# daeheepark/TrajSDE

Measured on AMD Instinct MI355X. Metric: scenes/sec (K=6, 20 SDE steps, ~256 agents) at 1/2/4/8 MI355X; minADE match, higher is better.
Workload: dtype f32 (fp16x3 split: 22-bit operands on v_mfma_f32_16x16x32_f16, f32 accumulate)

## Files before the change

### trajsde_amd/csrc/prep.hip

```cpp

#include <algorithm>
#include <cmath>
#include <limits>
#include <atomic>
#include <cstdlib>
#include <cstring>

#include "common.hpp"
#include "philox.hpp"
#include "tile.hpp"

namespace tsde {

__global__ void k_rotate(const float* __restrict__ ang, int N, const float* __restrict__ y, int F,
                         float* __restrict__ rot, float* __restrict__ y_rot) {
  const int per = F > 0 && y != nullptr ? F : 1;
  const int64_t idx = int64_t(blockIdx.x) * blockDim.x + threadIdx.x;
  if (idx >= int64_t(N) * per) return;
  const int i = int(idx / per), t = int(idx - int64_t(i) * per);
  const float s = sinf(ang[i]), c = cosf(ang[i]);
  if (t == 0) {
    f4 r = {c, -s, s, c};
    *reinterpret_cast<f4*>(rot + 4 * i) = r;
  }
  if (y != nullptr && F > 0) {
    const float a = y[(int64_t(i) * F + t) * 2], b = y[(int64_t(i) * F + t) * 2 + 1];
    y_rot[(int64_t(i) * F + t) * 2] = a * c + b * s;
    y_rot[(int64_t(i) * F + t) * 2 + 1] = b * c - a * s;
  }
}


constexpr int DONE_WAYS = 16;
__device__ __forceinline__ bool last_block_done(unsigned int* counters , unsigned int total) {
  __shared__ int s_last;
  asm volatile("s_waitcnt vmcnt(0)" ::: "memory");
  __syncthreads();
  if (threadIdx.x == 0) {
    const unsigned way = blockIdx.x % DONE_WAYS;
    const unsigned quota = total / DONE_WAYS + (way < total % DONE_WAYS ? 1u : 0u);
    int last = 0;
    if (__hip_atomic_fetch_add(&counters[way], 1u, __ATOMIC_RELAXED, __HIP_MEMORY_SCOPE_AGENT) + 1u == quota) {
      unsigned ways_used = total < unsigned(DONE_WAYS) ? total : unsigned(DONE_WAYS);
      last = __hip_atomic_fetch_add(&counters[DONE_WAYS], 1u, __ATOMIC_RELAXED, __HIP_MEMORY_SCOPE_AGENT) + 1u == ways_used;
    }
    s_last = last;
  }
  __syncthreads();
  return s_last != 0;
}
struct CoherentI32 {
  __amdgpu_buffer_rsrc_t rs;
  __device__ __forceinline__ explicit CoherentI32(const int32_t* base)
      : rs(__builtin_amdgcn_make_buffer_rsrc(const_cast<int32_t*>(base), 0, 0xFFFFFFFF, 0x00020000)) {}
  __device__ __forceinline__ int32_t operator[](int i) const { return __builtin_amdgcn_raw_buffer_load_b32(rs, i * 4, 0, 16 ); }
};
__device__ __forceinline__ void store_through(int32_t* p, int32_t v) { __hip_atomic_store(p, v, __ATOMIC_RELAXED, __HIP_MEMORY_SCOPE_AGENT); }

constexpr int EPT = 16;
__device__ __forceinline__ void degree_body(int blk, const int64_t* __restrict__ ei, int E, int32_t* __restrict__ deg) {
  int d[EPT];
#pragma unroll
  for (int u = 0; u < EPT; ++u) {
    const int e = (blk * EPT + u) * 256 + int(threadIdx.x);
    d[u] = e < E ? int(ei[int64_t(E) + e]) : -1;
  }
#pragma unroll
  for (int u = 0; u < EPT; ++u)
    if (d[u] >= 0) atomicAdd(&deg[d[u]], 1);
}
__device__ __forceinline__ void scatter_body(int blk, const int64_t* __restrict__ ei, int E, const int32_t* __restrict__ rowptr,
                                             int32_t* __restrict__ deg, int32_t* __restrict__ out) {
  int d[EPT], p[EPT], src[EPT];
#pragma unroll
  for (int u = 0; u < EPT; ++u) {
    const int e = (blk * EPT + u) * 256 + int(threadIdx.x);
    d[u] = e < E ? int(ei[int64_t(E) + e]) : -1;
    src[u] = e < E ? int32_t(ei[e]) : 0;
  }
#pragma unroll
  for (int u = 0; u < EPT; ++u) p[u] = d[u] >= 0 ? rowptr[d[u]] + atomicSub(&deg[d[u]], 1) - 1 : -1;
#pragma unroll
  for (int u = 0; u < EPT; ++u)
    if (p[u] >= 0) out[p[u]] = src[u];
}
__device__ __forceinline__ void scatter_lane_body(int blk, const int64_t* __restrict__ lai, int E, const int32_t* __restrict__ rowptr,
                                                  int32_t* __restrict__ deg, int64_t* __restrict__ out) {
  int d[EPT], p[EPT];
  int64_t key[EPT];
#pragma unroll
  for (int u = 0; u < EPT; ++u) {
    const int e = (blk * EPT + u) * 256 + int(threadIdx.x);
    d[u] = e < E ? int(lai[int64_t(E) + e]) : -1;
    key[u] = e < E ? ((lai[e] << 32) | int64_t(e)) : 0;
  }
#pragma unroll
  for (int u = 0; u < EPT; ++u) p[u] = d[u] >= 0 ? rowptr[d[u]] + atomicSub(&deg[d[u]], 1) - 1 : -1;
#pragma unroll
  for (int u = 0; u < EPT; ++u)
    if (p[u] >= 0) out[p[u]] = key[u];
}
__global__ __launch_bounds__(256) void k_scatter2(const int64_t* __restrict__ ei, int E, const int32_t* __restrict__ rowptr, int32_t* __restrict__ deg,
                                                  int32_t* __restrict__ csr_src, int nb_a, const int64_t* __restrict__ lai, int Ea,
                                                  const int32_t* __restrict__ la_rowptr, int32_t* __restrict__ la_deg, int64_t* __restrict__ la_pack) {
  const int blk = blockIdx.x;
  if (blk < nb_a) scatter_body(blk, ei, E, rowptr, deg, csr_src);
  else scatter_lane_body(blk - nb_a, lai, Ea, la_rowptr, la_deg, la_pack);
}
template <typename T, typename EMIT>
__device__ __forceinline__ void sort_long_rows(int vblk, int vgrid, const int32_t* __restrict__ rowptr, int n_rows, T* __restrict__ vals,
                                               T* buf , int32_t* __restrict__ low_out, int32_t* __restrict__ row_out,
                                               const EMIT& emit) {
  const T INF = sizeof(T) == 8 ? T(INT64_MAX) : T(INT32_MAX);
  for (int row = vblk; row < n_rows; row += vgrid) {
    const int beg = rowptr[row], n = rowptr[row + 1] - beg;
    if (n <= 256) continue;
    if (row_out != nullptr)
      for (int i = threadIdx.x; i < n; i += blockDim.x) row_out[beg + i] = row;
    int P = 2;
    while (P < n) P <<= 1;
    if (P <= 4096) {
      for (int i = threadIdx.x; i < P; i += blockDim.x) buf[i] = i < n ? vals[beg + i] : INF;
      __syncthreads();
      for (int k = 2; k <= P; k <<= 1)
        for (int j = k >> 1; j > 0; j >>= 1) {
          for (int i = threadIdx.x; i < P; i += blockDim.x) {
            const int l = i ^ j;
            if (l > i) {
              const T vi = buf[i], vl = buf[l];
              const bool up = (i & k) == 0;
              if ((vi > vl) == up) {
                buf[i] = vl;
                buf[l] = vi;
              }
            }
          }
          __syncthreads();
        }
      for (int i = threadIdx.x; i < n; i += blockDim.x) {
        vals[beg + i] = buf[i];
        if (low_out != nullptr) low_out[beg + i] = int32_t(int64_t(buf[i]) & 0xFFFFFFFFll);
        emit(beg + i, buf[i], row);
      }
      __syncthreads();
    } else {
      T* a = vals + beg;
      for (int k = 2; k <= P; k <<= 1)
        for (int j = k >> 1; j > 0; j >>= 1) {
          const int mask = (j == (k >> 1)) ? k - 1 : j;
          for (int i = threadIdx.x; i < n; i += blockDim.x) {
            const int l = i ^ mask;
            if (l > i && l < n) {
              const T vi = a[i], vl = a[l];
              if (vi > vl) {
                a[i] = vl;
                a[l] = vi;
              }
            }
          }
          __threadfence_block();
          __syncthreads();
        }
      for (int i = threadIdx.x; i < n; i += blockDim.x) {
        if (low_out != nullptr) low_out[beg + i] = int32_t(int64_t(a[i]) & 0xFFFFFFFFll);
        emit(beg + i, a[i], row);
      }
    }
  }
}

template <typename T>
__device__ __forceinline__ T lane_xor(T v, int mask) {
  if constexpr (sizeof(T) == 8) {
    const unsigned lo = unsigned(__shfl_xor(int(unsigned(v & 0xFFFFFFFFll)), mask)), hi = unsigned(__shfl_xor(int(unsigned((v >> 32) & 0xFFFFFFFFll)), mask));
    return T((int64_t(hi) << 32) | int64_t(lo));
  } else {
    return T(__shfl_xor(int(v), mask));
  }
}
template <typename T, typename EMIT>
__device__ __forceinline__ void row_sort_part(int vblk, int vgrid, const int32_t* __restrict__ rowptr, int n_rows, T* __restrict__ vals,
                                              int32_t* __restrict__ low_out ,
                                              int32_t* __restrict__ row_out ,
                                              T* buf , const EMIT& emit) {
  constexpr int EPL = 4, PMAX = 64 * EPL;
  const T INF = sizeof(T) == 8 ? T(INT64_MAX) : T(INT32_MAX);
  const int lane = threadIdx.x & 63, waves = blockDim.x >> 6;
  for (int row = vblk * waves + (threadIdx.x >> 6); row < n_rows; row += vgrid * waves) {
    const int beg = rowptr[row], n = rowptr[row + 1] - beg;
    if (n > PMAX) continue;
    if (row_out != nullptr) {
#pragma unroll
      for (int r = 0; r < EPL; ++r)
        if (64 * r + lane < n) row_out[beg + 64 * r + lane] = row;
    }
    if (n <= 1) {
      if (n == 1 && lane == 0) {
        const T v0 = vals[beg];
        if (low_out != nullptr) low_out[beg] = int32_t(int64_t(v0) & 0xFFFFFFFFll);
        emit(beg, v0, row);
      }
      continue;
    }
    T v[EPL];
#pragma unroll
    for (int r = 0; r < EPL; ++r) v[r] = EPL * lane + r < n ? vals[beg + EPL * lane + r] : INF;
#pragma unroll
    for (int k = 2; k <= PMAX; k <<= 1) {
      if ((k >> 1) >= n) break;
#pragma unroll
      for (int j = k >> 1; j > 0; j >>= 1) {
        if (j < EPL) {
#pragma unroll
          for (int r = 0; r < EPL; ++r) {
            const int l = r ^ j;
            if (l > r) {
              const bool up = ((EPL * lane + r) & k) == 0;
              const T a = v[r], b = v[l];
              const bool sw = (a > b) == up;
              v[r] = sw ? b : a;
              v[l] = sw ? a : b;
            }
          }
        } else {
          const int lj = j / EPL;
          const bool lower = (lane & lj) == 0;
#pragma unroll
          for (int r = 0; r < EPL; ++r) {
            const T o = lane_xor<T>(v[r], lj);
            const bool up = ((EPL * lane + r) & k) == 0;
            const bool keep_min = lower == up;
            v[r] = keep_min ? (o < v[r] ? o : v[r]) : (o > v[r] ? o : v[r]);
          }
        }
      }
    }
#pragma unroll
    for (int r = 0; r < EPL; ++r)
      if (EPL * lane + r < n) {
        vals[beg + EPL * lane + r] = v[r];
        if (low_out != nullptr) low_out[beg + EPL * lane + r] = int32_t(int64_t(v[r]) & 0xFFFFFFFFll);
        emit(beg + EPL * lane + r, v[r], row);
      }
  }
  sort_long_rows<T>(vblk, vgrid, rowptr, n_rows, vals, buf, low_out, row_out, emit);
}

__device__ __forceinline__ void ext_nodes_body(int i, int N, int A, int H, const int64_t* __restrict__ agent_index,
                                               const int64_t* __restrict__ batch, const int64_t* __restrict__ source,
                                               const uint8_t* __restrict__ bos, int32_t* __restrict__ orig, uint8_t* __restrict__ nus,
                                               int32_t* __restrict__ eos, int32_t* __restrict__ pick_slot) {
  __shared__ int32_t s_agents[256];
  int slot = -1;
  for (int k0 = 0; k0 < A; k0 += 256) {
    __syncthreads();
    s_agents[threadIdx.x] = k0 + int(threadIdx.x) < A ? int32_t(agent_index[k0 + threadIdx.x]) : -1;
    __syncthreads();
    const int m = A - k0 < 256 ? A - k0 : 256;
    if (i < N)
      for (int k = 0; k < m; ++k)
        if (s_agents[k] == i) slot = k0 + k;
  }
  if (i >= N + A) return;
  const int o = i < N ? i : int(agent_index[i - N]);
  orig[i] = o;
  nus[i] = (i < N ? source[batch[i]] : source[i - N]) == 0;
  int first = 0;
  {
    uint8_t bv[32];
#pragma unroll
    for (int t = 0; t < 32; ++t) bv[t] = bos[int64_t(o) * H + (t < H ? t : H - 1)];
#pragma unroll
    for (int t = 31; t >= 0; --t)
      if (t < H && bv[t]) first = t;
  }
  eos[i] = (H - 1) - first;
  pick_slot[i] = i < N ? slot : A + (i - N);
}

__device__ __forceinline__ void fake_x_body(int idx , int A, int H, const float* __restrict__ x,
                                            const int64_t* __restrict__ agent_index, const NoiseArg& na, float* __restrict__ x_fake) {
  const int quads = (2 * H + 3) / 4;
  if (idx >= A * quads) return;
  const int k = idx / quads, q = idx % quads;
  f4 z;
  if (na.z != nullptr) {
    for (int c = 0; c < 4; ++c) z[c] = (4 * q + c < 2 * H) ? na.z[int64_t(k) * 2 * H + 4 * q + c] : 0.f;
  } else {
    z = philox_normal4(noise_key(na), STREAM_FAKE_AGENT, 0u, na.row_ids ? uint32_t(na.row_ids[k]) : uint32_t(k), uint32_t(q));
  }
  const int64_t a = agent_index[k];
  for (int c = 0; c < 4; ++c) {
    const int col = 4 * q + c;
    if (col < 2 * H) x_fake[int64_t(k) * 2 * H + col] = x[a * 2 * H + col] + 2.0f * z[c];
  }
}

__device__ __forceinline__ float norm2_sq(float dx, float dy) { return fmaf(dy, dy, __fmul_rn(dx, dx)); }
__device__ __forceinline__ bool within_radius2(float dx, float dy, float thr2) { return norm2_sq(dx, dy) < thr2; }
static float radius2_threshold(float radius) {
  if (!(radius > 0.f)) return 0.f;
  if (std::isinf(radius)) return radius;
  float t = radius * radius;
  if (std::isinf(t)) t = std::numeric_limits<float>::max();
  while (t > 0.f && std::sqrt(t) >= radius) t = std::nextafter(t, 0.f);
  while (std::sqrt(t) < radius) t = std::nextafter(t, std::numeric_limits<float>::infinity());
  return t;
}

__device__ __forceinline__ void valid_mask_body(int i, int N, int H, int TT, const uint8_t* __restrict__ pad, uint32_t* __restrict__ vmask) {
  if (i >= N) return;
  uint32_t m = 0;
  uint8_t v[32];
#pragma unroll
  for (int t = 0; t < 32; ++t) v[t] = pad[int64_t(i) * TT + (t < H ? t : H - 1)];
#pragma unroll
  for (int t = 0; t < 32; ++t) m |= uint32_t(t < H && !v[t]) << t;
  vmask[i] = m;
}
__device__ __forceinline__ void time_major_body(int blk, int N, int H, int TT, const float* __restrict__ pos,
                                                const float* __restrict__ x, float2* __restrict__ pos_t, float2* __restrict__ x_t) {
  float2 pv[4], xv[4];
  int ii[4], tt[4];
#pragma unroll
  for (int u = 0; u < 4; ++u) {
    const int idx = (blk * 4 + u) * 256 + int(threadIdx.x);
    const bool live = idx < N * H;
    ii[u] = live ? idx / H : -1;
    tt[u] = live ? idx - ii[u] * H : 0;
    pv[u] = live ? reinterpret_cast<const float2*>(pos)[int64_t(ii[u]) * TT + tt[u]] : float2{0.f, 0.f};
    xv[u] = live ? reinterpret_cast<const float2*>(x)[int64_t(ii[u]) * H + tt[u]] : float2{0.f, 0.f};
  }
#pragma unroll
  for (int u = 0; u < 4; ++u)
    if (ii[u] >= 0) {
      pos_t[int64_t(tt[u]) * N + ii[u]] = pv[u];
      x_t[int64_t(tt[u]) * N + ii[u]] = xv[u];
    }
}

__device__ __forceinline__ void lane_feat_body(int l, int L, int P, const float* __restrict__ lp, const float* __restrict__ pad,
                                               float* __restrict__ feat) {
  if (l >= L) return;
  float len = 0.f;
  for (int j0 = 0; j0 < P; j0 += 8) {
    float pv[8];
#pragma unroll
    for (int u = 0; u < 8; ++u) pv[u] = pad[int64_t(l) * P + (j0 + u < P ? j0 + u : P - 1)];
#pragma unroll
    for (int u = 0; u < 8; ++u)
      if (j0 + u < P) len += 1.0f - pv[u];
  }
  int last = int(len - 1.0f);
  if (last < 0) last += P;
  feat[2 * l] = lp[(int64_t(l) * P + last) * 2] - lp[int64_t(l) * P * 2];
  feat[2 * l + 1] = lp[(int64_t(l) * P + last) * 2 + 1] - lp[int64_t(l) * P * 2 + 1];
}

__device__ __forceinline__ void block_scan_two(const int32_t* __restrict__ in0, int32_t* __restrict__ out0, const int32_t* __restrict__ in1,
                                               int32_t* __restrict__ out1, int n) {
  __shared__ int32_t s_w[2][4];
  __shared__ int32_t s_carry[2];
  constexpr int PT = 32;
  const int t = threadIdx.x, lane = t & 63, wv = t >> 6;
  if (t < 2) s_carry[t] = 0;
  __syncthreads();
  const CoherentI32 c0(in0), c1(in1);
  for (int base = 0; base < n; base += 256 * PT) {
    int32_t v[2][PT], sum[2] = {0, 0};
#pragma unroll
    for (int c = 0; c < PT; ++c) {
      const int i = base + PT * t + c;
      v[0][c] = i < n ? c0[i] : 0;
      v[1][c] = i < n ? c1[i] : 0;
    }
#pragma unroll
    for (int c = 0; c < PT; ++c) {
      sum[0] += v[0][c];
      sum[1] += v[1][c];
    }
    int32_t inc[2] = {sum[0], sum[1]};
#pragma unroll
    for (int d = 1; d < 64; d <<= 1) {
      const int32_t o0 = __shfl_up(inc[0], d), o1 = __shfl_up(inc[1], d);
      if (lane >= d) { inc[0] += o0; inc[1] += o1; }
    }
    if (lane == 63) { s_w[0][wv] = inc[0]; s_w[1][wv] = inc[1]; }
    __syncthreads();
#pragma unroll
    for (int a = 0; a < 2; ++a) {
      int32_t run = s_carry[a] + inc[a] - sum[a];
      for (int w = 0; w < wv; ++w) run += s_w[a][w];
      int32_t* out = a ? out1 : out0;
#pragma unroll
      for (int c = 0; c < PT; ++c) {
        const int i = base + PT * t + c;
        if (i < n) out[i] = run;
        run += v[a][c];
      }
    }
    __syncthreads();
    if (t < 2) s_carry[t] += s_w[t][0] + s_w[t][1] + s_w[t][2] + s_w[t][3];
    __syncthreads();
  }
}

struct FirstPassArgs {
  int N, A, H, TT, L, P, E, Ea, b0, b1, b2, b3, b4, b5, blocks;
  const int64_t *edge_index, *lane_actor_index, *agent_index, *batch, *source;
  const uint8_t *bos, *pad;
  const float *x, *pos, *lane_pos, *lane_pad;
  int32_t *deg, *la_deg, *rowptr, *la_rowptr, *orig, *eos, *pick_slot;
  uint8_t* nus;
  float *x_fake, *lane_feat;
  float2 *pos_t, *x_t;
  uint32_t* vmask;
  unsigned int* done;
  NoiseArg na;
};
__global__ __launch_bounds__(256) void k_prep_first(const FirstPassArgs a) {
  const int blk = blockIdx.x, i = threadIdx.x;
  if (blk < a.b0) degree_body(blk, a.edge_index, a.E, a.deg);
  else if (blk < a.b1) degree_body(blk - a.b0, a.lane_actor_index, a.Ea, a.la_deg);
  else if (blk < a.b2) ext_nodes_body((blk - a.b1) * 256 + i, a.N, a.A, a.H, a.agent_index, a.batch, a.source, a.bos, a.orig, a.nus, a.eos, a.pick_slot);
  else if (blk < a.b3) fake_x_body((blk - a.b2) * 256 + i, a.A, a.H, a.x, a.agent_index, a.na, a.x_fake);
  else if (blk < a.b4) valid_mask_body((blk - a.b3) * 256 + i, a.N, a.H, a.TT, a.pad, a.vmask);
  else if (blk < a.b5) time_major_body(blk - a.b4, a.N, a.H, a.TT, a.pos, a.x, a.pos_t, a.x_t);
  else lane_feat_body((blk - a.b5) * 256 + i, a.L, a.P, a.lane_pos, a.lane_pad, a.lane_feat);
  if (!last_block_done(a.done, unsigned(a.blocks))) return;
  block_scan_two(a.deg, a.rowptr, a.la_deg, a.la_rowptr, a.N + 1);
}

__global__ __launch_bounds__(256) void k_row_sort2(int N, int nb_a, int nb_l, const int32_t* __restrict__ rowptr, int32_t* __restrict__ csr_src,
                                                   int32_t* __restrict__ csr_dst, const uint32_t* __restrict__ vmask, int tref, int E,
                                                   uint8_t* __restrict__ flags_g, const int32_t* __restrict__ la_rowptr,
                                                   int64_t* __restrict__ la_pack, int32_t* __restrict__ la_eid, int32_t* __restrict__ la_actor,
                                                   const float* __restrict__ vec, float radius, int Ea, uint8_t* __restrict__ flags_la) {
  __shared__ int64_t buf[4096];
  const int blk = blockIdx.x;
  if (blk == 0 && threadIdx.x == 0) {
    flags_g[E] = 0;
    flags_la[Ea] = 0;
  }
  if (blk < nb_a) {
    if (E <= 0) return;
    auto emit = [&](int p, int32_t sender, int row) { flags_g[p] = uint8_t((vmask[sender] >> tref) & (vmask[row] >> tref) & 1u); };
    row_sort_part<int32_t>(blk, nb_a, rowptr, N, csr_src, nullptr, csr_dst, reinterpret_cast<int32_t*>(buf), emit);
  } else {
    if (Ea <= 0) return;
    auto emit = [&](int p, int64_t packed, int row) {
      (void)row;
      const int64_t e = packed & 0xFFFFFFFFll;
      flags_la[p] = uint8_t(sqrtf(norm2_sq(vec[2 * e], vec[2 * e + 1])) < radius);
    };
    row_sort_part<int64_t>(blk - nb_a, nb_l, la_rowptr, N, la_pack, la_eid, la_actor, buf, emit);
  }
}

constexpr int SCAN_MAX_BLOCKS = 512;
constexpr int SCAN_WORDS = SCAN_MAX_BLOCKS + 1;
constexpr int SCAN_INSTANCES = 3;
__device__ __forceinline__ int32_t lookback_prefix(unsigned long long* __restrict__ words, int b, int32_t total, int lane) {
  if (lane == 0)
    __hip_atomic_store(&words[b], ((b == 0 ? 2ull : 1ull) << 32) | (unsigned long long)(unsigned)total, __ATOMIC_RELAXED, __HIP_MEMORY_SCOPE_AGENT);
  int32_t prefix = 0;
  if (b > 0) {
    int j = b - 1;
    for (long spins = 0;; ++spins) {
      if (spins > (1L << 28)) __builtin_trap();
      const int k = j - lane;
      const unsigned long long w = k >= 0 ? __hip_atomic_load(&words[k], __ATOMIC_RELAXED, __HIP_MEMORY_SCOPE_AGENT) : (2ull << 32);
      const unsigned flag = unsigned(w >> 32);
      const unsigned long long done = __ballot(flag == 2u), none = __ballot(flag == 0u);
      const int upto = done ? __builtin_ctzll(done) : 63;
      const unsigned long long need = upto == 63 ? ~0ull : ((1ull << (upto + 1)) - 1);
      if (none & need) continue;
      int32_t part = lane <= upto ? int32_t(unsigned(w)) : 0;
#pragma unroll
      for (int d = 1; d < 64; d <<= 1) part += __shfl_xor(part, d);
      prefix += part;
      if (done) break;
      j -= 64;
    }
    if (lane == 0)
      __hip_atomic_store(&words[b], (2ull << 32) | (unsigned long long)(unsigned)(prefix + total), __ATOMIC_RELAXED, __HIP_MEMORY_SCOPE_AGENT);
  }
  return prefix;
}
struct ScanJob {
  const void* in;
  int32_t* out;
  int n, u8, blocks;
  unsigned long long* st;
};
struct ScanMultiArgs {
  ScanJob j[3];
  int njobs, blocks;
};
template <int PER>
__global__ __launch_bounds__(1024) void k_scan_multi(const ScanMultiArgs a) {
  __shared__ int32_t wsum[16];
  __shared__ int s_bid;
  __shared__ int32_t s_prefix;
  const int t = threadIdx.x, lane = t & 63, wv = t >> 6;
  int blk = blockIdx.x, q = 0;
  while (q + 1 < a.njobs && blk >= a.j[q].blocks) { blk -= a.j[q].blocks; ++q; }
  const ScanJob& job = a.j[q];
  const int n = job.n;
  if (t == 0) s_bid = int(__hip_atomic_fetch_add(&job.st[0], 1ull, __ATOMIC_RELAXED, __HIP_MEMORY_SCOPE_AGENT));
  __syncthreads();
  const int b = s_bid;
  const int64_t first = (int64_t(b) * 1024 + t) * PER;
  int32_t v[PER];
  int32_t s = 0;
#pragma unroll
  for (int i = 0; i < PER; ++i) {
    v[i] = first + i < n ? (job.u8 ? int32_t(static_cast<const uint8_t*>(job.in)[first + i]) : static_cast<const int32_t*>(job.in)[first + i]) : 0;
    s += v[i];
  }
  int32_t inc = s;
#pragma unroll
  for (int d = 1; d < 64; d <<= 1) {
    const int32_t o = __shfl_up(inc, d);
    if (lane >= d) inc += o;
  }
  if (lane == 63) wsum[wv] = inc;
  __syncthreads();
  int32_t wbase = 0;
  for (int w = 0; w < wv; ++w) wbase += wsum[w];
  if (wv == 0) {
    int32_t total = lane < 16 ? wsum[lane] : 0;
#pragma unroll
    for (int d = 1; d < 16; d <<= 1) total += __shfl_xor(total, d);
    total = __shfl(total, 0);
    const int32_t prefix = lookback_prefix(job.st + 1, b, total, lane);
    if (lane == 0) s_prefix = prefix;
  }
  __syncthreads();
  int32_t run = s_prefix + wbase + inc - s;
#pragma unroll
  for (int i = 0; i < PER; ++i) {
    if (first + i < n) job.out[first + i] = run;
    run += v[i];
  }
}
struct CollectArgs {
  int64_t n_aa;
  int E, Ea, N;
  const int32_t *aa_segptr, *cpos_g, *cpos_la, *rowptr, *la_rowptr;
  int32_t *g_segptr, *la_segptr, *counts;
  float radius, thr2;
  int radius_dev;
};
__device__ __forceinline__ void collect_body(int i, const CollectArgs& a) {
  if (i <= a.N) {
    a.g_segptr[i] = a.cpos_g[a.rowptr[i]];
    a.la_segptr[i] = a.cpos_la[a.la_rowptr[i]];
  }
  if (i == 0) {
    a.counts[0] = 0;
    a.counts[1] = a.aa_segptr[a.n_aa];
    a.counts[2] = a.cpos_g[a.E];
    a.counts[3] = a.cpos_la[a.Ea];
    if (!a.radius_dev) reinterpret_cast<float*>(a.counts)[4] = a.radius;
  }
}
__global__ void k_collect_counts(const CollectArgs a) { collect_body(blockIdx.x * blockDim.x + threadIdx.x, a); }

struct AaArgs {
  int N, Nt, H;
  float radius, thr2;
  int thr2_dev;
  const int32_t *rowptr, *csr_src, *orig;
  const uint32_t* vmask;
  const float2 *pos_t, *x_t;
  const float* rot;
  int32_t* segptr;
  int32_t* counts;
  unsigned long long* bal;
  int32_t *aa_dst, *aa_src;
  float* geom;
};
__device__ __forceinline__ int64_t bal_base(int row_start, int o) { return int64_t(row_start >> 6) + o; }
__device__ __forceinline__ int nth_set_bit(unsigned long long w, int r) {
  int posn = 0;
#pragma unroll
  for (int width = 32; width >= 1; width >>= 1) {
    const int c = __popcll((w >> posn) & ((1ull << width) - 1ull));
    if (r >= c) { r -= c; posn += width; }
  }
  return posn;
}
constexpr int AA_CG = 4, AA_SG = 7;
__global__ __launch_bounds__(256) void k_aa_count(const AaArgs a) {
  const int lane = threadIdx.x & 63;
  const int N = a.N, Nt = a.Nt, H = a.H;
  const int wid = __builtin_amdgcn_readfirstlane(int(xcd_block() * 4 + (threadIdx.x >> 6)));
  const int groups = (H + AA_SG - 1) / AA_SG, node = wid / groups, t0 = (wid - node * groups) * AA_SG;
  if (wid == 0 && lane == 0) {
    a.segptr[int64_t(H) * Nt] = 0;
    reinterpret_cast<float*>(a.counts)[4] = a.radius;
    reinterpret_cast<float*>(a.counts)[5] = a.thr2;
  }
  if (node >= Nt) return;
  const int o = node < N ? node : __builtin_amdgcn_readfirstlane(a.orig[node]);
  const int beg = __builtin_amdgcn_readfirstlane(a.rowptr[o]), end = __builtin_amdgcn_readfirstlane(a.rowptr[o + 1]);
  const uint32_t vo = __builtin_amdgcn_readfirstlane(a.vmask[o]);
  const int chunks = (end - beg + 63) >> 6;
  const int64_t bbase = bal_base(beg, o);
  const float thr2 = a.thr2;
  int mycnt = 0;
  for (int c0 = 0; c0 < chunks; c0 += AA_CG) {
    int s[AA_CG];
    uint32_t m[AA_CG];
#pragma unroll
    for (int u = 0; u < AA_CG; ++u) {
      const int p = beg + 64 * (c0 + u) + lane;
      s[u] = p < end ? a.csr_src[p] : -1;
    }
#pragma unroll
    for (int u = 0; u < AA_CG; ++u) {
      m[u] = s[u] >= 0 ? (a.vmask[s[u]] & vo) : 0u;
      s[u] = s[u] >= 0 ? s[u] : 0;
    }
    unsigned long long mine[AA_CG];
#pragma unroll
    for (int u = 0; u < AA_CG; ++u) mine[u] = 0ull;
    {
      float2 ps[AA_CG][AA_SG], pd[AA_SG];
#pragma unroll
      for (int q = 0; q < AA_SG; ++q) {
        const int t = t0 + q < H ? t0 + q : H - 1;
        pd[q] = a.pos_t[int64_t(t) * N + o];
#pragma unroll
        for (int u = 0; u < AA_CG; ++u) ps[u][q] = a.pos_t[int64_t(t) * N + s[u]];
      }
#pragma unroll
      for (int q = 0; q < AA_SG; ++q) {
        const int t = t0 + q;
        if (t >= H) break;
#pragma unroll
        for (int u = 0; u < AA_CG; ++u) {
          const bool ok = ((m[u] >> t) & 1u) && within_radius2(ps[u][q].x - pd[q].x, ps[u][q].y - pd[q].y, thr2);
          const unsigned long long B = __ballot(ok);
          mine[u] = lane == t ? B : mine[u];
        }
      }
    }
#pragma unroll
    for (int u = 0; u < AA_CG; ++u)
      if (c0 + u < chunks && lane >= t0 && lane < t0 + AA_SG && lane < H) {
        if (node < N) a.bal[(bbase + c0 + u) * H + lane] = mine[u];
        mycnt += __popcll(mine[u]);
      }
  }
  if (lane >= t0 && lane < t0 + AA_SG && lane < H) a.segptr[int64_t(lane) * Nt + node] = mycnt;
}
__device__ __forceinline__ void aa_fill_node(const AaArgs& a, int node, int part, int parts, int lane) {
  const int N = a.N, Nt = a.Nt, H = a.H;
  const int o = node < N ? node : __builtin_amdgcn_readfirstlane(a.orig[node]);
  const int beg = __builtin_amdgcn_readfirstlane(a.rowptr[o]), end = __builtin_amdgcn_readfirstlane(a.rowptr[o + 1]);
  if (end <= beg) return;
  const int chunks = (end - beg + 63) >> 6;
  const unsigned long long* __restrict__ words = a.bal + bal_base(beg, o) * H;
  int base_l = 0, n_l = 0;
  float2 pd_l = {0.f, 0.f};
  if (lane < H) {
    base_l = a.segptr[int64_t(lane) * Nt + node];
    n_l = a.segptr[int64_t(lane) * Nt + node + 1] - base_l;
    pd_l = a.pos_t[int64_t(lane) * N + o];
  }
  const int nw = chunks * H;
  const bool in_regs = nw <= 128;
  unsigned long long w0 = 0ull, w1 = 0ull;
  if (in_regs) {
    if (lane < nw) w0 = words[lane];
    if (64 + lane < nw) w1 = words[64 + lane];
  }
  const f4 R = *reinterpret_cast<const f4*>(a.rot + 4 * o);
  auto word = [&](int c, int t) -> unsigned long long {
    if (in_regs) {
      const int i = c * H + t;
      const unsigned long long src = i < 64 ? w0 : w1;
      const unsigned lo_ = __builtin_amdgcn_readlane(unsigned(src), i & 63), hi_ = __builtin_amdgcn_readlane(unsigned(src >> 32), i & 63);
      return (static_cast<unsigned long long>(hi_) << 32) | lo_;
    }
    return words[int64_t(c) * H + t];
  };
  for (int t = part; t < H; t += parts) {
    const int n = __builtin_amdgcn_readlane(n_l, t);
    if (n == 0) continue;
    const int64_t base = __builtin_amdgcn_readlane(base_l, t);
    const float pdx = __builtin_bit_cast(float, __builtin_amdgcn_readlane(__builtin_bit_cast(int, pd_l.x), t));
    const float pdy = __builtin_bit_cast(float, __builtin_amdgcn_readlane(__builtin_bit_cast(int, pd_l.y), t));
    const float2* __restrict__ pos_t = a.pos_t + int64_t(t) * N;
    const float2* __restrict__ x_t = a.x_t + int64_t(t) * N;
    const int seg = t * Nt + node;
    for (int r0 = 0; r0 < n; r0 += 64) {
      const int r = r0 + lane;
      unsigned long long selw = 0ull;
      int selc = 0, rr = 0, cum = 0;
      for (int c = 0; c < chunks; ++c) {
        const unsigned long long w = word(c, t);
        const int cc = __popcll(w);
        if (r >= cum && r < cum + cc) { selw = w; selc = c; rr = r - cum; }
        cum += cc;
        if (cum >= r0 + 64) break;
      }
      if (r < n) {
        const int sdr = a.csr_src[beg + 64 * selc + nth_set_bit(selw, rr)];
        const float2 ps = pos_t[sdr], xs = x_t[sdr];
        const float dx = ps.x - pdx, dy = ps.y - pdy;
        const float x0 = xs.x, x1 = xs.y;
        const f4 g = {x0 * R[0] + x1 * R[2], x0 * R[1] + x1 * R[3], dx * R[0] + dy * R[2], dx * R[1] + dy * R[3]};
        const int64_t k = base + r;
        *reinterpret_cast<f4*>(a.geom + 4 * k) = g;
        a.aa_dst[k] = seg;
        if (a.aa_src != nullptr) a.aa_src[k] = sdr;
      }
    }
  }
}

__device__ __forceinline__ void g_compact_body(int p, int E, int TT, int tref, const int32_t* __restrict__ csr_src, const int32_t* __restrict__ csr_dst,
                                               const float* __restrict__ pos, const float* __restrict__ rot, const float* __restrict__ ang,
                                               const uint8_t* __restrict__ flags, const int32_t* __restrict__ cpos, int32_t* __restrict__ g_src,
                                               int32_t* __restrict__ g_dst, float* __restrict__ geom) {
  if (p >= E || !flags[p]) return;
  const int s = csr_src[p], i = csr_dst[p], q = cpos[p];
  const f4 R = *reinterpret_cast<const f4*>(rot + 4 * i);
  const float dx = pos[(int64_t(s) * TT + tref) * 2] - pos[(int64_t(i) * TT + tref) * 2];
  const float dy = pos[(int64_t(s) * TT + tref) * 2 + 1] - pos[(int64_t(i) * TT + tref) * 2 + 1];
  const float th = ang[s] - ang[i];
  f4 g = {dx * R[0] + dy * R[2], dx * R[1] + dy * R[3], cosf(th), sinf(th)};
  *reinterpret_cast<f4*>(geom + 4 * int64_t(q)) = g;
  g_src[q] = s;
  g_dst[q] = i;
}
__device__ __forceinline__ void la_compact_body(int p, int E_al, const int32_t* __restrict__ actor, const int32_t* __restrict__ eid,
                                                const int64_t* __restrict__ la_index, const float* __restrict__ vec,
                                                const float* __restrict__ lane_feat, const float* __restrict__ rot,
                                                const uint8_t* __restrict__ flags, const int32_t* __restrict__ cpos, int32_t* __restrict__ la_dst,
                                                int32_t* __restrict__ la_lane, float* __restrict__ geom) {
  if (p >= E_al || !flags[p]) return;
  const int i = actor[p], e = eid[p], q = cpos[p];
  const int lane = int(la_index[e]);
  const f4 R = *reinterpret_cast<const f4*>(rot + 4 * i);
  const float fx = lane_feat[2 * lane], fy = lane_feat[2 * lane + 1], vx = vec[2 * int64_t(e)], vy = vec[2 * int64_t(e) + 1];
  f4 g = {fx * R[0] + fy * R[2], fx * R[1] + fy * R[3], vx * R[0] + vy * R[2], vx * R[1] + vy * R[3]};
  *reinterpret_cast<f4*>(geom + 4 * int64_t(q)) = g;
  la_dst[q] = i;
  if (la_lane != nullptr) la_lane[q] = lane;
}
struct FillArgs {
  AaArgs aa;
  CollectArgs col;
  int nb_c;
  int nb_g, nb_l, nb_a, parts;
  int E, TT, tref, Ea;
  const int32_t *csr_src, *csr_dst, *cpos_g, *la_actor, *la_eid, *cpos_la;
  const float *pos, *rot, *ang, *vec, *lane_feat;
  const uint8_t *flags_g, *flags_la;
  const int64_t* la_index;
  int32_t *g_src, *g_dst, *la_dst, *la_lane;
  float *g_geom, *la_geom;
};
__global__ __launch_bounds__(256) void k_graph_fill(const FillArgs f) {
  int blk = blockIdx.x;
  if (blk < f.nb_c) {
    collect_body(blk * 256 + threadIdx.x, f.col);
    return;
  }
  blk -= f.nb_c;
  if (blk < f.nb_g) {
    g_compact_body(blk * 256 + threadIdx.x, f.E, f.TT, f.tref, f.csr_src, f.csr_dst, f.pos, f.rot, f.ang, f.flags_g, f.cpos_g, f.g_src, f.g_dst, f.g_geom);
  } else if (blk < f.nb_g + f.nb_l) {
    la_compact_body((blk - f.nb_g) * 256 + threadIdx.x, f.Ea, f.la_actor, f.la_eid, f.la_index, f.vec, f.lane_feat, f.rot, f.flags_la, f.cpos_la,
                    f.la_dst, f.la_lane, f.la_geom);
  } else {
    const int ab = blk - f.nb_g - f.nb_l, logical = (ab & 7) * (f.nb_a >> 3) + (ab >> 3);
    const int wid = __builtin_amdgcn_readfirstlane(logical * 4 + int(threadIdx.x >> 6));
    const int node = wid / f.parts, part = wid - node * f.parts;
    if (node < f.aa.Nt) aa_fill_node(f.aa, node, part, f.parts, threadIdx.x & 63);
  }
}

struct PrepWs {
  int32_t *deg, *rowptr, *csr_src, *csr_dst, *orig, *eos, *pick_slot, *counts;
  int32_t *la_deg, *la_rowptr, *la_eid, *la_actor;
  int64_t* la_pack;
  int32_t *aa_segptr, *g_segptr, *la_segptr, *cpos_g, *cpos_la;
  uint8_t *nus, *flags_g, *flags_la;
  uint32_t* vmask;
  float2 *pos_t, *x_t;
  unsigned long long* bal;
  float *x_fake, *lane_feat;
  unsigned long long* scan_st;
  unsigned int* done;
  int64_t zeroed_bytes, n_aa, aa_blocks;
  int64_t total;
  bool ok;
  PrepWs(const trajsde_batch* b, void* ws, int64_t ws_bytes) {
    Carver c(ws, ws_bytes);
    const int64_t N = b->N, A = b->A, E = b->E, Nt = N + A, H = b->H, Ea = b->E_al;
    n_aa = H * Nt;
    aa_blocks = xcd_grid((Nt * ((H + 6) / 7) + 3) / 4);
    const int64_t deg_ints = (2 * (N + 1) + 1) / 2 * 2;
    const int64_t st_words = int64_t(SCAN_INSTANCES) * SCAN_WORDS + (DONE_WAYS + 2) / 2 + 1;
    deg = c.take<int32_t>(deg_ints + 2 * st_words); la_deg = ptr_add(deg, N + 1);
    scan_st = reinterpret_cast<unsigned long long*>(ptr_add(deg, deg_ints));
    done = reinterpret_cast<unsigned int*>(ptr_add(scan_st, int64_t(SCAN_INSTANCES) * SCAN_WORDS));
    zeroed_bytes = (deg_ints + 2 * st_words) * int64_t(sizeof(int32_t));
    rowptr = c.take<int32_t>(N + 1);
    csr_src = c.take<int32_t>(E + 1); csr_dst = c.take<int32_t>(E + 1);
    orig = c.take<int32_t>(Nt); eos = c.take<int32_t>(Nt); pick_slot = c.take<int32_t>(Nt); counts = c.take<int32_t>(8);
    la_rowptr = c.take<int32_t>(N + 1);
    la_eid = c.take<int32_t>(Ea + 1); la_actor = c.take<int32_t>(Ea + 1); la_pack = c.take<int64_t>(Ea + 1);
    aa_segptr = c.take<int32_t>(n_aa + 1); g_segptr = c.take<int32_t>(N + 1); la_segptr = c.take<int32_t>(N + 1);
    cpos_g = c.take<int32_t>(E + 1); cpos_la = c.take<int32_t>(Ea + 1);
    nus = c.take<uint8_t>(Nt); flags_g = c.take<uint8_t>(E + 1); flags_la = c.take<uint8_t>(Ea + 1);
    x_fake = c.take<float>(A * H * 2 + 4); lane_feat = c.take<float>(int64_t(b->L) * 2 + 4);
    vmask = c.take<uint32_t>(N + 1);
    pos_t = c.take<float2>(H * N + 1); x_t = c.take<float2>(H * N + 1);
    bal = c.take<unsigned long long>(((E >> 6) + N + 2) * H);
    total = c.off + 256;
    ok = c.ok;
  }
};

struct EdgeWs {
  float *aa_geom, *g_geom, *la_geom;
  int32_t *aa_dst, *aa_src, *g_src, *g_dst, *la_dst, *la_lane;
  int64_t total;
  bool ok;
  EdgeWs(const trajsde_batch* b, const trajsde_graph* g, void* ws, int64_t ws_bytes) {
    Carver c(ws, ws_bytes);
    (void)b;
    const int64_t Eaa = g->E_aa, Eg = g->E_g, Ela = g->E_la;
    aa_geom = c.take<float>(4 * Eaa + 4); aa_dst = c.take<int32_t>(Eaa + 1); aa_src = c.take<int32_t>(Eaa + 1);
    g_geom = c.take<float>(4 * Eg + 4); g_src = c.take<int32_t>(Eg + 1); g_dst = c.take<int32_t>(Eg + 1);
    la_geom = c.take<float>(4 * Ela + 4); la_dst = c.take<int32_t>(Ela + 1); la_lane = c.take<int32_t>(Ela + 1);
    total = c.off + 256;
    ok = c.ok;
  }
};

static int check_batch(const trajsde_batch* b) {
  TS_REQUIRE(b != nullptr, "batch: null");
  TS_REQUIRE(b->N > 0 && b->A >= 0 && b->H > 0 && b->H <= 32 && b->TT >= b->H, "batch: bad sizes (H <= 32)");
  TS_REQUIRE(b->E >= 0 && b->E_al >= 0 && b->L >= 0, "batch: negative sizes");
  TS_REQUIRE(int64_t(b->H) * b->E < (int64_t(1) << 31) - 2, "batch: too many (t, edge) candidates for int32 positions");
  TS_REQUIRE(b->x && b->positions && b->padding_mask && b->bos_mask && b->rotate_angles && b->batch && b->source,
             "batch: null actor tensor");
  TS_REQUIRE(b->A == 0 || b->agent_index, "batch: null agent_index");
  TS_REQUIRE(b->E == 0 || b->edge_index, "batch: null edge_index");
  TS_REQUIRE(b->E_al == 0 || (b->lane_actor_index && b->lane_actor_vectors && b->lane_positions && b->lane_paddings),
             "batch: null lane tensor");
  return TRAJSDE_OK;
}

static CollectArgs collect_args(const trajsde_batch* b, const PrepWs& w, float radius) {
  CollectArgs c;
  c.n_aa = w.n_aa; c.E = b->E; c.Ea = b->E_al; c.N = b->N;
  c.aa_segptr = w.aa_segptr; c.cpos_g = w.cpos_g; c.cpos_la = w.cpos_la; c.rowptr = w.rowptr; c.la_rowptr = w.la_rowptr;
  c.g_segptr = w.g_segptr; c.la_segptr = w.la_segptr; c.counts = w.counts; c.radius = radius; c.thr2 = 0.f; c.radius_dev = 0;
  return c;
}
static AaArgs aa_args(const trajsde_batch* b, const PrepWs& w, const float* rot, float radius) {
  AaArgs a;
  a.N = b->N; a.Nt = b->N + b->A; a.H = b->H;
  a.radius = radius; a.thr2 = radius2_threshold(radius); a.thr2_dev = 0;
  a.rowptr = w.rowptr; a.csr_src = w.csr_src; a.orig = w.orig; a.vmask = w.vmask; a.pos_t = w.pos_t; a.x_t = w.x_t; a.rot = rot;
  a.segptr = w.aa_segptr; a.counts = w.counts; a.bal = w.bal;
  a.aa_dst = nullptr; a.aa_src = nullptr; a.geom = nullptr;
  return a;
}

}

using namespace tsde;

static std::atomic<int> g_export_senders{0};

extern "C" {

float trajsde_radius2_threshold(float radius) { return radius2_threshold(radius); }

int trajsde_export_senders(int on) {
  const int prev = g_export_senders.exchange(on ? 1 : 0);
  return prev;
}

int trajsde_rotate(const float* rotate_angles, int32_t N, const float* y, int32_t F, float* rotate_mat, float* y_rot, void* stream) {
  TS_REQUIRE(rotate_angles && rotate_mat && N > 0, "rotate: bad argument");
  TS_REQUIRE(y == nullptr || y_rot != nullptr, "rotate: y given without y_rot");
  k_rotate<<<cdiv(int64_t(N) * (y != nullptr && F > 0 ? F : 1), 256), 256, 0, static_cast<hipStream_t>(stream)>>>(rotate_angles, N, y, F, rotate_mat, y_rot);
  TS_LAUNCH_CHECK("k_rotate");
  return TRAJSDE_OK;
}

int64_t trajsde_graph_ws_bytes(const trajsde_batch* b) {
  if (check_batch(b) != TRAJSDE_OK) return -1;
  PrepWs w(b, nullptr, 0);
  return w.total;
}

static int graph_prepare(const trajsde_batch* b, const float* rot, float radius, const trajsde_noise* fake_noise, void* ws,
                         int64_t ws_bytes, trajsde_graph* out, void* stream_, bool sync) {
  if (int rc = check_batch(b)) return rc;
  TS_REQUIRE(rot && ws && out, "graph_prepare: null pointer");
  PrepWs w(b, ws, ws_bytes);
  if (!w.ok) return fail(TRAJSDE_ERR_WORKSPACE, "graph_prepare: workspace too small");
  hipStream_t st = static_cast<hipStream_t>(stream_);
  const int N = b->N, A = b->A, E = b->E, H = b->H, TT = b->TT, Ea = b->E_al, Nt = N + A;
  NoiseArg na{0, nullptr, nullptr};
  if (fake_noise) { na.seed = fake_noise->seed; na.z = fake_noise->z; na.row_ids = fake_noise->row_ids; na.seed_dev = fake_noise->seed_dev; }

  TS_HIP(hipMemsetAsync(w.deg, 0, size_t(w.zeroed_bytes), st));
  const int tref = H - 1;
  {
    ProfScope ps("k_prep_first", st);
    FirstPassArgs fa;
    fa.N = N; fa.A = A; fa.H = H; fa.TT = TT; fa.L = b->L; fa.P = b->lane_pts; fa.E = E; fa.Ea = Ea;
    fa.b0 = cdiv(E, 256 * EPT);
    fa.b1 = fa.b0 + cdiv(Ea, 256 * EPT);
    fa.b2 = fa.b1 + cdiv(Nt, 256);
    fa.b3 = fa.b2 + (A > 0 ? cdiv(A * ((2 * H + 3) / 4), 256) : 0);
    fa.b4 = fa.b3 + cdiv(N, 256);
    fa.b5 = fa.b4 + cdiv(int64_t(N) * H, 1024);
    fa.blocks = fa.b5 + (b->L > 0 ? cdiv(b->L, 256) : 0);
    fa.edge_index = b->edge_index; fa.lane_actor_index = b->lane_actor_index; fa.agent_index = b->agent_index; fa.batch = b->batch;
    fa.source = b->source; fa.bos = b->bos_mask; fa.pad = b->padding_mask; fa.x = b->x; fa.pos = b->positions;
    fa.lane_pos = b->lane_positions; fa.lane_pad = b->lane_paddings;
    fa.deg = w.deg; fa.la_deg = w.la_deg; fa.rowptr = w.rowptr; fa.la_rowptr = w.la_rowptr; fa.orig = w.orig; fa.eos = w.eos;
    fa.pick_slot = w.pick_slot; fa.nus = w.nus; fa.x_fake = w.x_fake; fa.lane_feat = w.lane_feat; fa.pos_t = w.pos_t; fa.x_t = w.x_t;
    fa.vmask = w.vmask; fa.done = w.done + 0; fa.na = na;
    k_prep_first<<<fa.blocks, 256, 0, st>>>(fa);
  }
  if (E > 0 || Ea > 0) {
    ProfScope ps("k_scatter2", st);
    const int nb_a = cdiv(E, 256 * EPT);
    k_scatter2<<<nb_a + cdiv(Ea, 256 * EPT), 256, 0, st>>>(b->edge_index, E, w.rowptr, w.deg, w.csr_src, nb_a, b->lane_actor_index, Ea, w.la_rowptr,
                                                     w.la_deg, w.la_pack);
  }
  {
    ProfScope ps("k_row_sort2", st);
    const int per_list = cdiv(N, 4) < 8192 ? cdiv(N, 4) : 8192;
    k_row_sort2<<<2 * per_list, 256, 0, st>>>(N, per_list, per_list, w.rowptr, w.csr_src, w.csr_dst, w.vmask, tref, E, w.flags_g, w.la_rowptr,
                                              w.la_pack, w.la_eid, w.la_actor, b->lane_actor_vectors, radius, Ea, w.flags_la);
  }
  {
    ProfScope ps("k_aa_count", st);
    const AaArgs aa = aa_args(b, w, rot, radius);
    k_aa_count<<<int(w.aa_blocks), 256, 0, st>>>(aa);
  }
  {
    ProfScope ps("k_scan_multi", st);
    ScanMultiArgs sa;
    std::memset(&sa, 0, sizeof(sa));
    int64_t nmax = 0;
    auto add = [&](const void* in, int32_t* out_, int64_t n, int u8, int inst) {
      ScanJob& j = sa.j[sa.njobs++];
      j.in = in; j.out = out_; j.n = int(n); j.u8 = u8; j.st = w.scan_st + int64_t(inst) * SCAN_WORDS;
      nmax = std::max(nmax, n);
    };
    add(w.aa_segptr, w.aa_segptr, w.n_aa + 1, 0, 0);
    add(w.flags_g, w.cpos_g, int64_t(E) + 1, 1, 1);
    add(w.flags_la, w.cpos_la, int64_t(Ea) + 1, 1, 2);
    TS_REQUIRE(nmax <= int64_t(SCAN_MAX_BLOCKS) * 65536, "graph stage: more than 33 M elements in a prefix sum");
    const int64_t per = (nmax + int64_t(SCAN_MAX_BLOCKS) * 1024 - 1) / (int64_t(SCAN_MAX_BLOCKS) * 1024);
    const int PER = per <= 8 ? 8 : (per <= 16 ? 16 : (per <= 32 ? 32 : 64));
    for (int q = 0; q < sa.njobs; ++q) {
      sa.j[q].blocks = cdiv(sa.j[q].n, PER * 1024);
      sa.blocks += sa.j[q].blocks;
    }
    if (PER == 8) k_scan_multi<8><<<sa.blocks, 1024, 0, st>>>(sa);
    else if (PER == 16) k_scan_multi<16><<<sa.blocks, 1024, 0, st>>>(sa);
    else if (PER == 32) k_scan_multi<32><<<sa.blocks, 1024, 0, st>>>(sa);
    else k_scan_multi<64><<<sa.blocks, 1024, 0, st>>>(sa);
  }
  if (sync) {
    ProfScope ps("k_collect_counts", st);
    k_collect_counts<<<cdiv(N + 1, 256), 256, 0, st>>>(collect_args(b, w, radius));
  }
  TS_LAUNCH_CHECK("graph_prepare kernels");
  int32_t h[4] = {0, 0, 0, 0};
  if (sync) {
    TS_HIP(hipMemcpyAsync(h, w.counts, sizeof(h), hipMemcpyDeviceToHost, st));
    TS_HIP(hipStreamSynchronize(st));
  } else {
    const int64_t aa_max = int64_t(H) * 2 * int64_t(E);
    (void)A;
    TS_REQUIRE(aa_max < (int64_t(1) << 31) - 2, "graph_prepare_async: too many (t, edge) candidates for int32 positions");
    h[1] = int32_t(aa_max); h[2] = E; h[3] = Ea;
  }
  std::memset(out, 0, sizeof(*out));
  out->counts = w.counts; out->exact = sync ? 1 : 0;
  out->Nt = Nt; out->E_ext = E; out->E_aa = h[1]; out->E_g = h[2]; out->E_la = h[3];
  out->orig = w.orig; out->nus_mask = w.nus; out->eos_idx = w.eos; out->pick_slot = w.pick_slot; out->x_fake = w.x_fake;
  out->aa_segptr = w.aa_segptr; out->g_segptr = w.g_segptr; out->la_segptr = w.la_segptr;
  return TRAJSDE_OK;
}

int trajsde_graph_prepare(const trajsde_batch* b, const float* rot, float radius, const trajsde_noise* fake_noise, void* ws,
                          int64_t ws_bytes, trajsde_graph* out, void* stream_) {
  return graph_prepare(b, rot, radius, fake_noise, ws, ws_bytes, out, stream_, true);
}

int trajsde_graph_prepare_async(const trajsde_batch* b, const float* rot, float radius, const trajsde_noise* fake_noise, void* ws,
                                int64_t ws_bytes, trajsde_graph* out, void* stream_) {
  return graph_prepare(b, rot, radius, fake_noise, ws, ws_bytes, out, stream_, false);
}

int64_t trajsde_graph_edges_ws_bytes(const trajsde_batch* b, const trajsde_graph* g) {
  if (!b || !g) return -1;
  EdgeWs e(b, g, nullptr, 0);
  return e.total;
}

int trajsde_graph_compact(const trajsde_batch* b, const float* rot, void* ws, int64_t ws_bytes, void* edges_ws,
                          int64_t edges_ws_bytes, trajsde_graph* out, void* stream_) {
  if (int rc = check_batch(b)) return rc;
  TS_REQUIRE(rot && ws && edges_ws && out, "graph_compact: null pointer");
  PrepWs w(b, ws, ws_bytes);
  EdgeWs e(b, out, edges_ws, edges_ws_bytes);
  if (!w.ok || !e.ok) return fail(TRAJSDE_ERR_WORKSPACE, "graph_compact: workspace too small");
  hipStream_t st = static_cast<hipStream_t>(stream_);
  const int E = b->E, H = b->H, TT = b->TT, Ea = b->E_al;
  const bool want_src = g_export_senders.load() != 0;
  {
    ProfScope ps("k_graph_fill", st);
    FillArgs f;
    f.aa = aa_args(b, w, rot, 0.f);
    f.aa.aa_dst = e.aa_dst; f.aa.aa_src = want_src ? e.aa_src : nullptr; f.aa.geom = e.aa_geom;
    f.nb_g = cdiv(E, 256); f.nb_l = cdiv(Ea, 256);
    f.E = E; f.TT = TT; f.tref = H - 1; f.Ea = Ea;
    f.csr_src = w.csr_src; f.csr_dst = w.csr_dst; f.cpos_g = w.cpos_g; f.la_actor = w.la_actor; f.la_eid = w.la_eid; f.cpos_la = w.cpos_la;
    f.pos = b->positions; f.rot = rot; f.ang = b->rotate_angles; f.vec = b->lane_actor_vectors; f.lane_feat = w.lane_feat;
    f.flags_g = w.flags_g; f.flags_la = w.flags_la; f.la_index = b->lane_actor_index;
    f.g_src = e.g_src; f.g_dst = e.g_dst; f.la_dst = e.la_dst; f.la_lane = want_src ? e.la_lane : nullptr;
    f.g_geom = e.g_geom; f.la_geom = e.la_geom;
    f.col = collect_args(b, w, 0.f);
    f.col.radius_dev = 1;
    f.nb_c = out->exact ? 0 : cdiv(b->N + 1, 256);
    const bool aa_work = E > 0 && out->E_aa > 0;
    static const int fill_parts = []() { const char* e = getenv("TRAJSDE_FILL_PARTS"); const int v = e ? atoi(e) : 3; return v >= 1 && v <= 32 ? v : 3; }();
    f.parts = fill_parts;
    f.nb_a = xcd_grid(cdiv(int64_t(b->N + b->A) * f.parts, 4));
    const int blocks = f.nb_c + f.nb_g + f.nb_l + (aa_work ? f.nb_a : 0);
    if (blocks > 0) k_graph_fill<<<blocks, 256, 0, st>>>(f);
  }
  TS_LAUNCH_CHECK("graph_compact kernels");
  out->aa_geom = e.aa_geom; out->aa_dst = e.aa_dst;
  out->aa_src = want_src ? e.aa_src : nullptr; out->la_lane = want_src ? e.la_lane : nullptr;
  out->g_geom = e.g_geom; out->g_src = e.g_src; out->g_dst = e.g_dst;
  out->la_geom = e.la_geom; out->la_dst = e.la_dst;
  return TRAJSDE_OK;
}

}
```

Before: 16160.

## Cache sender indices in registers for agent-agent fill and read transposed positions

```diff
diff --git a/trajsde_amd/csrc/prep.hip b/trajsde_amd/csrc/prep.hip
--- a/trajsde_amd/csrc/prep.hip
+++ b/trajsde_amd/csrc/prep.hip
@@ -656,81 +656,148 @@
   }
   if (lane >= t0 && lane < t0 + AA_SG && lane < H) a.segptr[int64_t(lane) * Nt + node] = mycnt;
 }
+#ifndef TSDE_FILL_SC
+#define TSDE_FILL_SC 4
+#endif
+#ifndef TSDE_FILL_SETTLE
+#define TSDE_FILL_SETTLE 1
+#endif
+constexpr int FILL_SC = TSDE_FILL_SC;
+static_assert(FILL_SC >= 0 && FILL_SC <= 4, "a row whose senders fit the registers must have its ballot words in registers too: 4 x 32 <= 128");
+struct FillRound {
+  int t, r0;
+  int sdr;
+  float2 ps, xs;
+};
+struct FillRow {
+  int node, o, beg, chunks;
+  int base_l, n_l;
+  float2 pd_l;
+  unsigned long long w0, w1;
+  bool in_regs;
+  const unsigned long long* words;
+  int sreg[FILL_SC > 0 ? FILL_SC : 1];
+  f4 R;
+};
+template <bool REGS>
+__device__ __forceinline__ void aa_fill_rounds(const AaArgs& a, const FillRow& w, int part, int parts, int lane) {
+  const int N = a.N, Nt = a.Nt, H = a.H;
+  const int chunks = w.chunks;
+  auto word = [&](int c, int t) -> unsigned long long {
+    if (REGS || w.in_regs) {
+      const int i = c * H + t;
+      const unsigned long long src = i < 64 ? w.w0 : w.w1;
+      const unsigned lo_ = __builtin_amdgcn_readlane(unsigned(src), i & 63), hi_ = __builtin_amdgcn_readlane(unsigned(src >> 32), i & 63);
+      return (static_cast<unsigned long long>(hi_) << 32) | lo_;
+    }
+    return w.words[int64_t(c) * H + t];
+  };
+  auto next_step = [&](int t) -> int {
+    while (t < H && __builtin_amdgcn_readlane(w.n_l, t) == 0) t += parts;
+    return t < H ? t : H;
+  };
+  auto request = [&](int t, int r0) -> FillRound {
+    const int n = __builtin_amdgcn_readlane(w.n_l, t);
+    const int r = r0 + lane;
+    unsigned long long selw = 0ull;
+    int selc = 0, rr = 0, cum = 0;
+    for (int c = 0; c < chunks; ++c) {
+      const unsigned long long bw = word(c, t);
+      const int cc = __popcll(bw);
+      if (r >= cum && r < cum + cc) { selw = bw; selc = c; rr = r - cum; }
+      cum += cc;
+      if (cum >= r0 + 64) break;
+    }
+    const int bit = r < n ? nth_set_bit(selw, rr) : 0;
+    FillRound q;
+    q.t = t; q.r0 = r0; q.sdr = 0;
+    if (REGS) {
+#pragma unroll
+      for (int u = 0; u < FILL_SC; ++u) {
+        const int v = __builtin_amdgcn_ds_bpermute(bit << 2, w.sreg[u]);
+        q.sdr = selc == u ? v : q.sdr;
+      }
+    } else {
+      q.sdr = a.csr_src[w.beg + 64 * selc + bit];
+    }
+    q.ps = a.pos_t[int64_t(t) * N + q.sdr];
+    q.xs = a.x_t[int64_t(t) * N + q.sdr];
+    return q;
+  };
+  auto finish = [&](const FillRound& q) {
+    const int t = q.t, r = q.r0 + lane;
+    const int n = __builtin_amdgcn_readlane(w.n_l, t);
+    const int64_t base = __builtin_amdgcn_readlane(w.base_l, t);
+    const float pdx = __builtin_bit_cast(float, __builtin_amdgcn_readlane(__builtin_bit_cast(int, w.pd_l.x), t));
+    const float pdy = __builtin_bit_cast(float, __builtin_amdgcn_readlane(__builtin_bit_cast(int, w.pd_l.y), t));
+    if (r < n) {
+      const float dx = q.ps.x - pdx, dy = q.ps.y - pdy;
+      const float x0 = q.xs.x, x1 = q.xs.y;
+      const f4 R = w.R;
+      const f4 g = {fmaf(x0, R[0], __fmul_rn(x1, R[2])), fmaf(x0, R[1], __fmul_rn(x1, R[3])), fmaf(dx, R[0], __fmul_rn(dy, R[2])),
+                    fmaf(dx, R[1], __fmul_rn(dy, R[3]))};
+      const int64_t k = base + r;
+      *reinterpret_cast<f4*>(a.geom + 4 * k) = g;
+      a.aa_dst[k] = t * Nt + w.node;
+      if (a.aa_src != nullptr) a.aa_src[k] = q.sdr;
+    }
+  };
+  for (int t = next_step(part); t < H; t = next_step(t + parts)) {
+    const int n = __builtin_amdgcn_readlane(w.n_l, t);
+    for (int r0 = 0; r0 < n; r0 += 64) finish(request(t, r0));
+  }
+}
 __device__ __forceinline__ void aa_fill_node(const AaArgs& a, int node, int part, int parts, int lane) {
   const int N = a.N, Nt = a.Nt, H = a.H;
-  const int o = node < N ? node : __builtin_amdgcn_readfirstlane(a.orig[node]);
+  FillRow w;
+  w.node = node;
+  w.o = node < N ? node : __builtin_amdgcn_readfirstlane(a.orig[node]);
+  const int o = w.o;
   const int beg = __builtin_amdgcn_readfirstlane(a.rowptr[o]), end = __builtin_amdgcn_readfirstlane(a.rowptr[o + 1]);
   if (end <= beg) return;
-  const int chunks = (end - beg + 63) >> 6;
-  const unsigned long long* __restrict__ words = a.bal + bal_base(beg, o) * H;
-  int base_l = 0, n_l = 0;
-  float2 pd_l = {0.f, 0.f};
+  w.beg = beg;
+  w.chunks = (end - beg + 63) >> 6;
+  w.words = a.bal + bal_base(beg, o) * H;
+  w.base_l = 0; w.n_l = 0;
+  w.pd_l = float2{0.f, 0.f};
   if (lane < H) {
-    base_l = a.segptr[int64_t(lane) * Nt + node];
-    n_l = a.segptr[int64_t(lane) * Nt + node + 1] - base_l;
-    pd_l = a.pos_t[int64_t(lane) * N + o];
-  }
-  const int nw = chunks * H;
-  const bool in_regs = nw <= 128;
-  unsigned long long w0 = 0ull, w1 = 0ull;
-  if (in_regs) {
-    if (lane < nw) w0 = words[lane];
-    if (64 + lane < nw) w1 = words[64 + lane];
-  }
-  const f4 R = *reinterpret_cast<const f4*>(a.rot + 4 * o);
-  auto word = [&](int c, int t) -> unsigned long long {
-    if (in_regs) {
-      const int i = c * H + t;
-      const unsigned long long src = i < 64 ? w0 : w1;
-      const unsigned lo_ = __builtin_amdgcn_readlane(unsigned(src), i & 63), hi_ = __builtin_amdgcn_readlane(unsigned(src >> 32), i & 63);
-      return (static_cast<unsigned long long>(hi_) << 32) | lo_;
-    }
-    return words[int64_t(c) * H + t];
-  };
-  for (int t = part; t < H; t += parts) {
-    const int n = __builtin_amdgcn_readlane(n_l, t);
-    if (n == 0) continue;
-    const int64_t base = __builtin_amdgcn_readlane(base_l, t);
-    const float pdx = __builtin_bit_cast(float, __builtin_amdgcn_readlane(__builtin_bit_cast(int, pd_l.x), t));
-    const float pdy = __builtin_bit_cast(float, __builtin_amdgcn_readlane(__builtin_bit_cast(int, pd_l.y), t));
-    const float2* __restrict__ pos_t = a.pos_t + int64_t(t) * N;
-    const float2* __restrict__ x_t = a.x_t + int64_t(t) * N;
-    const int seg = t * Nt + node;
-    for (int r0 = 0; r0 < n; r0 += 64) {
-      const int r = r0 + lane;
-      unsigned long long selw = 0ull;
-      int selc = 0, rr = 0, cum = 0;
-      for (int c = 0; c < chunks; ++c) {
-        const unsigned long long w = word(c, t);
-        const int cc = __popcll(w);
-        if (r >= cum && r < cum + cc) { selw = w; selc = c; rr = r - cum; }
-        cum += cc;
-        if (cum >= r0 + 64) break;
-      }
-      if (r < n) {
-        const int sdr = a.csr_src[beg + 64 * selc + nth_set_bit(selw, rr)];
-        const float2 ps = pos_t[sdr], xs = x_t[sdr];
-        const float dx = ps.x - pdx, dy = ps.y - pdy;
-        const float x0 = xs.x, x1 = xs.y;
-        const f4 g = {x0 * R[0] + x1 * R[2], x0 * R[1] + x1 * R[3], dx * R[0] + dy * R[2], dx * R[1] + dy * R[3]};
-        const int64_t k = base + r;
-        *reinterpret_cast<f4*>(a.geom + 4 * k) = g;
-        a.aa_dst[k] = seg;
-        if (a.aa_src != nullptr) a.aa_src[k] = sdr;
-      }
-    }
-  }
-}
-
-__device__ __forceinline__ void g_compact_body(int p, int E, int TT, int tref, const int32_t* __restrict__ csr_src, const int32_t* __restrict__ csr_dst,
-                                               const float* __restrict__ pos, const float* __restrict__ rot, const float* __restrict__ ang,
+    w.base_l = a.segptr[int64_t(lane) * Nt + node];
+    w.n_l = a.segptr[int64_t(lane) * Nt + node + 1] - w.base_l;
+    w.pd_l = a.pos_t[int64_t(lane) * N + o];
+  }
+  const int nw = w.chunks * H;
+  w.in_regs = nw <= 128;
+  w.w0 = 0ull; w.w1 = 0ull;
+  if (w.in_regs) {
+    if (lane < nw) w.w0 = w.words[lane];
+    if (64 + lane < nw) w.w1 = w.words[64 + lane];
+  }
+  const bool s_regs = FILL_SC > 0 && w.chunks <= FILL_SC;
+#pragma unroll
+  for (int u = 0; u < (FILL_SC > 0 ? FILL_SC : 1); ++u) {
+    const int p = beg + 64 * u + lane;
+    w.sreg[u] = s_regs && p < end ? a.csr_src[p] : 0;
+  }
+  w.R = *reinterpret_cast<const f4*>(a.rot + 4 * o);
+#if TSDE_FILL_SETTLE
+  asm volatile("" : "+v"(w.base_l), "+v"(w.n_l), "+v"(w.pd_l.x), "+v"(w.pd_l.y), "+v"(w.w0), "+v"(w.w1));
+#pragma unroll
+  for (int u = 0; u < (FILL_SC > 0 ? FILL_SC : 1); ++u) asm volatile("" : "+v"(w.sreg[u]));
+#endif
+  if (s_regs) aa_fill_rounds<true>(a, w, part, parts, lane);
+  else aa_fill_rounds<false>(a, w, part, parts, lane);
+}
+
+__device__ __forceinline__ void g_compact_body(int p, int E, int N, int tref, const int32_t* __restrict__ csr_src, const int32_t* __restrict__ csr_dst,
+                                               const float2* __restrict__ pos_t, const float* __restrict__ rot, const float* __restrict__ ang,
                                                const uint8_t* __restrict__ flags, const int32_t* __restrict__ cpos, int32_t* __restrict__ g_src,
                                                int32_t* __restrict__ g_dst, float* __restrict__ geom) {
   if (p >= E || !flags[p]) return;
   const int s = csr_src[p], i = csr_dst[p], q = cpos[p];
   const f4 R = *reinterpret_cast<const f4*>(rot + 4 * i);
-  const float dx = pos[(int64_t(s) * TT + tref) * 2] - pos[(int64_t(i) * TT + tref) * 2];
-  const float dy = pos[(int64_t(s) * TT + tref) * 2 + 1] - pos[(int64_t(i) * TT + tref) * 2 + 1];
+  const float2 ps = pos_t[int64_t(tref) * N + s], pi = pos_t[int64_t(tref) * N + i];
+  const float dx = ps.x - pi.x;
+  const float dy = ps.y - pi.y;
   const float th = ang[s] - ang[i];
   f4 g = {dx * R[0] + dy * R[2], dx * R[1] + dy * R[3], cosf(th), sinf(th)};
   *reinterpret_cast<f4*>(geom + 4 * int64_t(q)) = g;
@@ -773,7 +840,7 @@
   }
   blk -= f.nb_c;
   if (blk < f.nb_g) {
-    g_compact_body(blk * 256 + threadIdx.x, f.E, f.TT, f.tref, f.csr_src, f.csr_dst, f.pos, f.rot, f.ang, f.flags_g, f.cpos_g, f.g_src, f.g_dst, f.g_geom);
+    g_compact_body(blk * 256 + threadIdx.x, f.E, f.aa.N, f.tref, f.csr_src, f.csr_dst, f.aa.pos_t, f.rot, f.ang, f.flags_g, f.cpos_g, f.g_src, f.g_dst, f.g_geom);
   } else if (blk < f.nb_g + f.nb_l) {
     la_compact_body((blk - f.nb_g) * 256 + threadIdx.x, f.Ea, f.la_actor, f.la_eid, f.la_index, f.vec, f.lane_feat, f.rot, f.flags_la, f.cpos_la,
                     f.la_dst, f.la_lane, f.la_geom);
```

Result: no change. 16260, median of 6 (+0.7%).
